# unilight/seq2seq-vc

Measured on AMD Instinct MI355X. Metric: mel-frames/sec (train), higher is better.
Workload: dtype bf16; 1 GPU; VTN egs/arctic/vc1 (vtn.v1.yaml) training step: fwd+Seq2SeqLoss+bwd+clip+Adam+WarmupLR; batch_per_gpu=32, global_batch=32, T_src=256, T_tgt=256, mel_dim=80, parallelism=dp1, split_backward=False, hip_graph=True, backward_stages=1

## Files before the change

### include/s2svc_hip.h

```cpp
#ifndef S2SVC_HIP_H
#define S2SVC_HIP_H
#include <stdint.h>
#ifdef __cplusplus
extern "C" {
#endif

const char* s2svc_last_error(void);
int s2svc_abi_version(void);
int s2svc_launch_floor(int workgroups, int threads, void* sink_1024_words, void* stream);

int s2svc_event_create(void** out );
int s2svc_event_destroy(void* ev);
int s2svc_event_record(void* ev, void* stream);
int s2svc_stream_wait_event(void* stream, void* ev);

enum { S2SVC_LAYOUT_KC = 0,
       S2SVC_LAYOUT_RC = 1 };
enum { S2SVC_OP_DENSE = 0,
       S2SVC_OP_CONV1D = 1,
       S2SVC_OP_CONV2D_S2 = 2,
       S2SVC_OP_TCONV2D_S2 = 3 };

typedef struct {
  const void* ptr;
// ... 116 lines not shown
int s2svc_axpby(int dtype, int64_t n, float a, const void* x, float b, const void* y, void* out, void* stream);
#define S2SVC_SCALAR_TERMS_MAX 8
typedef struct {
  const float* x[S2SVC_SCALAR_TERMS_MAX];
  int32_t n[S2SVC_SCALAR_TERMS_MAX];
  float w[S2SVC_SCALAR_TERMS_MAX];
  int32_t k;
  int32_t reserved_;
} s2svc_scalar_terms;
int s2svc_weighted_sum(const s2svc_scalar_terms* terms , float* out, void* stream);
int s2svc_weighted_sum_bwd(const s2svc_scalar_terms* grads , const float* g, void* stream);
int s2svc_scalars_axpy(const s2svc_scalar_terms* terms , float beta, float* acc, void* stream);
int s2svc_fill_zero(void* p, int64_t nbytes, void* stream);
int s2svc_seed_advance(uint64_t* seed, uint64_t inc, void* stream);
int s2svc_pad_cols(int dtype, int64_t rows, int N, int ldo, const void* in, void* out, void* stream);
int s2svc_decoder_input(int out_dtype, int B, int Tin, int r, int D, int64_t ys_batch_stride, const float* ys, void* out, void* stream);
int s2svc_append_eos(int B, int T, int64_t ldx, const int64_t* xs, const int32_t* lens, int64_t eos, int64_t pad, int64_t* out, void* stream);
int s2svc_copy_rows(int dtype, int64_t rows, int D, int64_t lds, const void* src, void* out, void* stream);
int s2svc_stop_labels(int B, int T, int64_t ld_labels, const float* labels, const int32_t* lens, float* out, void* stream);
int s2svc_add_n(int dtype, int64_t n, int k, const void* x0, const void* x1, const void* x2, const void* x3, void* out, void* stream);
int s2svc_add_head_bias(int dtype, int64_t rows, int D, const void* q, const float* u, const float* v, void* qu, void* qv,
                        void* stream);
int s2svc_add_head_bias_ld(int dtype, int64_t rows, int D, const void* q, int64_t ldq, const float* u, const float* v, void* qu,
                           void* qv, void* stream);
int s2svc_add_rows(int dtype, int64_t rows, int D, const void* a, int64_t lda, const void* b, int64_t ldb, void* out, int64_t ldo,
                   void* stream);
int s2svc_glu_fwd(int dtype, int64_t rows, int C, const void* x, void* y, void* stream);
int s2svc_glu_bwd(int dtype, int64_t rows, int C, const void* x, const void* dy, void* dx, void* stream);
int s2svc_cast(int in_dtype, int out_dtype, int64_t n, const void* x, void* y, void* stream);
int s2svc_gather3(int in_dtype, int out_dtype, int n0, int n1, int n2, int64_t s0, int64_t s1, int64_t s2, int64_t off,
                  const void* in, void* out, void* stream);
typedef struct s2svc_gather3_job {
  const void* in;
  void* out;
  int64_t s0, s1, s2, off;
  int32_t n0, n1, n2;
  int32_t out_dtype;
} s2svc_gather3_job;
int s2svc_gather3_grouped(const s2svc_gather3_job* jobs , int n, void* stream);
enum { S2SVC_DERIVED_GATHER3 = 0, S2SVC_DERIVED_TCONV2D = 1 };
typedef struct s2svc_derived_job {
  const void* in;
  void* out;
  int64_t s0, s1, s2, off;
  int32_t n0, n1, n2;
  int32_t out_dtype;
  int32_t kind;
  int32_t reserved_;
} s2svc_derived_job;
int s2svc_derived_refresh(const s2svc_derived_job* jobs , int n, void* stream);
int s2svc_derived_refresh_plan(const s2svc_derived_job* jobs , int n, int32_t* path , int32_t* units );
int s2svc_permute_inner(int n, int A, int B, const float* src, float* dst, int accumulate, void* stream);
int s2svc_rowscale(int dtype, int64_t rows, int D, const void* x, const float* s, void* out, void* stream);

int s2svc_conv_in1_fwd(int dtype, int B, int Tn, int Fn, int O, const void* x, const float* w, const float* bias, void* y,
                       void* stream);
int s2svc_conv_in1_wgrad(int dtype, int B, int Tn, int Fn, int O, const void* x, const void* dy, const void* y, float* dw,
                         float* db, int accumulate, float* partial, int max_chunks, void* stream);
int s2svc_col2im_s2(int dtype, int B, int T1, int F1, int C, int T2, int F2, const void* dcols, void* dx, void* stream);
int s2svc_interp_nearest(int dtype, int B, int Tin, int Tout, int C, const void* x, void* y, const int32_t* ext_in,
                         const int32_t* ext_out, void* stream);
int s2svc_interp_nearest_bwd(int dtype, int B, int Tin, int Tout, int C, const void* dy, void* dx, const int32_t* ext_in,
                             const int32_t* ext_out, void* stream);
int s2svc_interp_nearest_rows(int dtype, int B, int Tin, int Tout, int C, const void* x, void* y, const int32_t* lens_in,
                              const int32_t* lens_out, void* stream);
int s2svc_dwconv(int dtype, int B, int Tn, int C, int ks, int dil, const void* x, const float* w, const float* bias,
                 void* y, int flip, void* stream);
int s2svc_dwconv_add(int dtype, int B, int Tn, int C, int ks, int dil, const void* x, const float* w, const float* bias,
                     const void* add, void* y, int flip, void* stream);
int s2svc_dwconv_wgrad(int dtype, int B, int Tn, int C, int ks, int dil, const void* x, const void* dy, float* dw,
                       int accumulate, float* ws, int ws_chunks, void* stream);

int s2svc_convmod_supported(int C, int ks);
int s2svc_convmod_fwd(int B, int Tn, int C, int ks, const void* y2, const float* w, const float* bias, void* z, float eps,
                      float momentum, float* mean, float* rstd, float* run_mean, float* run_var, int64_t* num_batches, float* ws,
                      const int32_t* vlens, void* stream);
int s2svc_bn_swish_apply(int64_t rows, int C, const void* z, const float* mean, const float* rstd, const float* gamma,
                         const float* beta, void* out, int Tn, const int32_t* vlens, void* stream);
int s2svc_convmod_bwd(int B, int Tn, int C, int ks, const void* da, const void* z, const void* y2, const float* w, const float* mean,
                      const float* rstd, const float* gamma, const float* beta, void* dy2, float* sdy, float* sdyx,
                      float* dgamma_acc, float* dbeta_acc, float* ws_stats, float* ws_w, const int32_t* vlens, void* stream);
int s2svc_convmod_wgrad_final(int C, int ks, int chunks, const float* ws_w, float* dw, float* db, int accumulate, void* stream);

int s2svc_convmod_infer_supported(int C, int ks);
int s2svc_convmod_infer(int dtype, int B, int Tn, int C, int ks, const void* y2, const float* w, const float* bias, const float* run_mean,
                        const float* run_var, const float* gamma, const float* beta, float eps, void* out, const int32_t* vlens,
                        void* stream);

int s2svc_bn_stats_vec(int rows, int C, const void* x, float eps, float momentum, float* mean, float* rstd, float* run_mean,
                       float* run_var, int64_t* num_batches, float* ws, int Tn, const int32_t* vlens, void* stream);
int s2svc_bn_act_apply_vec(int rows, int C, const void* x, const float* mean, const float* rstd, const float* gamma, const float* beta,
                           int act, float drop_p, const uint64_t* seed_base, uint64_t seed_off, void* y, void* pre_act, int Tn,
                           const int32_t* vlens, void* stream);
int s2svc_bn_act_bwd_vec(int rows, int C, const void* dz, const void* saved, const void* x, const float* mean, const float* rstd,
                         const float* gamma, int act, float drop_p, const uint64_t* seed_base, uint64_t seed_off, void* dx, float* sdy,
                         float* sdyx, float* dgamma_acc, float* dbeta_acc, float* ws, int Tn, const int32_t* vlens, void* stream);

int s2svc_pairwise_l2_logsoftmax(int dtype, int B, int Tf, int Tx, int A, const void* feats, const void* text,
                                 const int32_t* text_lens, float* logp, float* dist, void* stream);
int s2svc_pairwise_l2_bwd_g(int dtype, int B, int Tf, int Tx, const float* logp, const float* dist, const float* dlogp,
                            const int32_t* text_lens, void* G, float* rowsum, void* stream);
int64_t s2svc_mas_ws_bytes(int B, int Tf, int Tx);
int s2svc_mas(int B, int Tf, int Tx, const float* log_p_attn, const int32_t* text_lens, const int32_t* feat_lens,
              int32_t* path, float* ds, float* binmean, void* ws, void* stream);
int s2svc_mas_binloss_bwd(int B, int Tf, int Tx, const int32_t* path, const int32_t* feat_lens, const float* gout,
                          float* dlogp, void* stream);
// ... 189 lines not shown
```

### seq2seq_vc_amd/_lib.py

```python
import ctypes
import os
import subprocess
import sys
from concurrent.futures import ThreadPoolExecutor

_HERE = os.path.dirname(os.path.abspath(__file__))
CSRC = os.path.join(_HERE, "csrc")
LIB_PATH = os.environ.get("S2SVC_LIB") or os.path.join(CSRC, "libs2svc_hip.so")
HIPCC = os.environ.get("HIPCC", "/opt/rocm/bin/hipcc")
ARCH = "gfx950"


def sources():
    return sorted(f for f in os.listdir(CSRC) if f.endswith(".hip"))


DEBUG_EXEC_LIB_PATH = os.path.join(CSRC, "libs2svc_hip_dbgexec.so")


def build_library(force=False, verbose=True, debug_exec=False):
    lib_path = DEBUG_EXEC_LIB_PATH if debug_exec else LIB_PATH
    if not debug_exec and os.environ.get("S2SVC_LIB"):
        lib_path = os.path.join(CSRC, "libs2svc_hip.so")
    srcs = [os.path.join(CSRC, f) for f in sources()]
# ... 40 lines not shown
    deps = [src, os.path.join(_HERE, "..", "include", "s2svc_hip.h")]
    if not force and os.path.exists(TORCH_OPS_LIB_PATH) and os.path.getmtime(TORCH_OPS_LIB_PATH) >= max(os.path.getmtime(p) for p in deps):
        return TORCH_OPS_LIB_PATH
    tlib = E.library_paths()[0]
    cmd = ["g++", "-O2", "-std=c++17", "-fPIC", "-shared", "-D__HIP_PLATFORM_AMD__=1", "-DUSE_ROCM=1",
           f"-D_GLIBCXX_USE_CXX11_ABI={int(torch._C._GLIBCXX_USE_CXX11_ABI)}"]
    cmd += [f"-I{p}" for p in E.include_paths()] + ["-I/opt/rocm/include", src, "-o", TORCH_OPS_LIB_PATH,
                                                    f"-L{tlib}", "-ltorch", "-ltorch_cpu", "-lc10", "-lc10_hip", "-ltorch_hip",
                                                    f"-L{CSRC}", "-ls2svc_hip", "-Wl,-rpath,$ORIGIN", f"-Wl,-rpath,{tlib}"]
    if verbose:
        print("[s2svc build]", " ".join(cmd), file=sys.stderr)
    subprocess.run(cmd, check=True)
    return TORCH_OPS_LIB_PATH


c_i32, c_i64, c_f32, c_u64, c_vp = ctypes.c_int32, ctypes.c_int64, ctypes.c_float, ctypes.c_uint64, ctypes.c_void_p


class Operand(ctypes.Structure):
    _fields_ = [("ptr", c_vp), ("ld", c_i64), ("layout", c_i32), ("mode", c_i32), ("C", c_i32), ("T", c_i32),
                ("pad", c_i32), ("T1", c_i32), ("F1", c_i32), ("T2", c_i32), ("F2", c_i32), ("bs0", c_i64),
                ("bs1", c_i64), ("zero_padded", c_i32), ("reserved_", c_i32)]


class GemmDesc(ctypes.Structure):
    _fields_ = [("A", Operand), ("B", Operand), ("C", c_vp), ("ldc", c_i64), ("cbs0", c_i64), ("cbs1", c_i64),
                ("c_dtype", c_i32), ("bias", c_vp), ("res", c_vp), ("ldr", c_i64), ("rbs0", c_i64), ("rbs1", c_i64),
                ("M", c_i32), ("N", c_i32), ("K", c_i32), ("nb0", c_i32), ("nb1", c_i32), ("act", c_i32),
                ("alpha", c_f32), ("dtype", c_i32), ("accumulate", c_i32), ("splitk", c_i32), ("ws", c_vp),
                ("a_rowsum", c_vp), ("a_rowsum_ws", c_vp), ("a_rowsum_accumulate", c_i32), ("tile_hint", c_i32),
                ("emask", c_vp), ("ldm", c_i64), ("drop_p", c_f32), ("emask_mode", c_i32), ("seed_base", c_vp),
                ("seed_off", c_u64), ("c_map", c_i32), ("cm_T1", c_i32), ("cm_F1", c_i32), ("cm_Tc", c_i32), ("cm_Fc", c_i32),
                ("cm_pt", c_i32), ("cm_pf", c_i32), ("reserved3_", c_i32), ("c_pre", c_vp)]


class ScalarTerms(ctypes.Structure):
    _fields_ = [("x", c_vp * 8), ("n", c_i32 * 8), ("w", c_f32 * 8), ("k", c_i32), ("reserved_", c_i32)]


class Gather3Job(ctypes.Structure):
    _fields_ = [("in_", c_vp), ("out", c_vp), ("s0", c_i64), ("s1", c_i64), ("s2", c_i64), ("off", c_i64), ("n0", c_i32),
                ("n1", c_i32), ("n2", c_i32), ("out_dtype", c_i32)]


class DerivedJob(ctypes.Structure):
    _fields_ = [("in_", c_vp), ("out", c_vp), ("s0", c_i64), ("s1", c_i64), ("s2", c_i64), ("off", c_i64), ("n0", c_i32),
                ("n1", c_i32), ("n2", c_i32), ("out_dtype", c_i32), ("kind", c_i32), ("reserved_", c_i32)]


class ColreduceItem(ctypes.Structure):
    _fields_ = [("dy", c_vp), ("x", c_vp), ("mean", c_vp), ("rstd", c_vp), ("out_sum", c_vp), ("out_dot", c_vp), ("ws", c_vp),
                ("dtype", c_i32), ("rows", c_i32), ("D", c_i32), ("mode", c_i32), ("accumulate", c_i32), ("ws_chunks", c_i32),
                ("scale", c_f32), ("reserved_", c_i32)]


_SIGS = {
    "s2svc_gemm": [ctypes.POINTER(GemmDesc), c_vp],
    "s2svc_gemm_grouped_ok": [c_vp],
    "s2svc_tconv2d_weights": [c_i32, c_i32, c_vp, c_vp, c_vp],
    "s2svc_gemm_grouped": [c_vp, c_i32, c_i32, c_vp],
    "s2svc_gemm_grouped_batched": [c_vp, c_i32, c_vp],
    "s2svc_gemm_wgrad_ok": [c_vp],
    "s2svc_gemm_wgrad_grouped": [c_vp, c_i32, c_vp, c_vp],
    "s2svc_gemm_wgrad_grouped_bg": [c_vp, c_i32, c_vp, c_vp, c_i32],
    "s2svc_gemm_set_w8": [c_i32, c_i32],
    "s2svc_gemm_set_8ph": [c_i32],
    "s2svc_launch_floor": [c_i32, c_i32, c_vp, c_vp],
    "s2svc_event_create": [c_vp],
    "s2svc_event_destroy": [c_vp],
    "s2svc_event_record": [c_vp, c_vp],
    "s2svc_stream_wait_event": [c_vp, c_vp],
    "s2svc_decode_ln_linear_supported": [c_i32, c_i32, c_i32],
    "s2svc_decode_ln_linear": [ctypes.POINTER(GemmDesc), c_vp, c_vp, c_f32, c_vp, c_i64, c_vp],
    "s2svc_length_regulate_index": [c_i32, c_i32, c_i32, c_vp, c_vp, c_vp, c_vp, c_vp],
    "s2svc_length_regulate_fwd": [c_i32, c_i32, c_i32, c_i32, c_i32, c_vp, c_vp, c_f32, c_vp, c_vp],
    "s2svc_length_regulate_bwd": [c_i32, c_i32, c_i32, c_i32, c_i32, c_vp, c_vp, c_vp, c_vp, c_vp],
    "s2svc_attn_durations": [c_i32, c_i32, c_i32, c_vp, c_vp, c_vp, c_vp, c_vp],
    "s2svc_durations_finalize": [c_i32, c_i32, c_i32, c_vp, c_vp, c_f32, c_vp, c_vp, c_vp, c_vp],
    "s2svc_layernorm_fwd": [c_i32, c_i32, c_i32, c_vp, c_vp, c_f32, c_f32, c_vp, c_u64, c_vp, c_vp, c_f32, c_vp, c_vp, c_vp, c_vp, c_vp],
    "s2svc_layernorm_bwd": [c_i32, c_i32, c_i32, c_vp, c_vp, c_vp, c_vp, c_vp, c_vp, c_f32, c_f32, c_vp, c_u64, c_vp, c_vp, c_vp],
    "s2svc_layernorm_bwd_pg_chunks": [c_i32, c_i32, c_i32, c_vp, c_vp, c_vp, c_vp, c_vp, c_vp],
    "s2svc_layernorm_bwd_pg": [c_i32, c_i32, c_i32, c_vp, c_vp, c_vp, c_vp, c_vp, c_vp, c_f32, c_f32, c_vp, c_u64, c_vp, c_vp, c_vp, c_vp],
    "s2svc_colreduce_grouped": [c_vp, c_i32, c_vp],
    "s2svc_colreduce": [c_i32, c_i32, c_i32, c_i32, c_vp, c_vp, c_vp, c_vp, c_f32, c_vp, c_vp, c_i32, c_vp, c_i32, c_i32, c_vp, c_vp],
    "s2svc_bn_finalize": [c_i32, c_i32, c_f32, c_f32, c_vp, c_vp, c_vp, c_vp, c_vp, c_vp, c_i32, c_i32, c_vp, c_vp],
    "s2svc_rstd_from_var": [c_i32, c_f32, c_vp, c_vp, c_vp],
    "s2svc_bn_apply": [c_i32, c_i64, c_i32, c_vp, c_vp, c_vp, c_vp, c_vp, c_i32, c_f32, c_vp, c_u64, c_vp, c_vp, c_i32, c_vp, c_vp],
    "s2svc_bn_bwd": [c_i32, c_i64, c_i32, c_vp, c_vp, c_vp, c_vp, c_vp, c_vp, c_vp, c_i32, c_vp, c_i32, c_vp, c_vp],
    "s2svc_bn_stats": [c_i32, c_i32, c_i32, c_vp, c_f32, c_f32, c_vp, c_vp, c_vp, c_vp, c_vp, c_vp, c_i32, c_i32, c_vp, c_vp],
    "s2svc_attn_softmax_fwd": [c_i32, c_i32, c_i32, c_i32, c_i32, c_i32, c_vp, c_vp, c_i32, c_i32, c_i32, c_f32, c_vp, c_i32, c_f32,
                               c_vp, c_u64, c_vp, c_vp, c_vp],
    "s2svc_attn_softmax_bwd": [c_i32, c_i32, c_i32, c_i32, c_i32, c_i32, c_vp, c_vp, c_vp, c_f32, c_f32, c_vp, c_u64, c_vp, c_vp, c_i32,
                               c_i32, c_i32, c_vp],
    "s2svc_act_dropout_fwd": [c_i32, c_i64, c_vp, c_i32, c_f32, c_vp, c_u64, c_vp, c_vp],
    "s2svc_act_dropout_bwd": [c_i32, c_i64, c_vp, c_vp, c_i32, c_f32, c_vp, c_u64, c_vp, c_vp],
    "s2svc_posenc_fwd": [c_i32, c_i64, c_i32, c_i32, c_vp, c_f32, c_vp, c_vp, c_f32, c_vp, c_u64, c_vp, c_vp],
    "s2svc_posenc_bwd": [c_i32, c_i64, c_i32, c_i32, c_vp, c_f32, c_vp, c_f32, c_vp, c_u64, c_vp, c_vp, c_vp, c_vp],
    "s2svc_axpby": [c_i32, c_i64, c_f32, c_vp, c_f32, c_vp, c_vp, c_vp],
    "s2svc_add_n": [c_i32, c_i64, c_i32, c_vp, c_vp, c_vp, c_vp, c_vp, c_vp],
    "s2svc_weighted_sum": [ctypes.POINTER(ScalarTerms), c_vp, c_vp],
    "s2svc_weighted_sum_bwd": [ctypes.POINTER(ScalarTerms), c_vp, c_vp],
    "s2svc_scalars_axpy": [ctypes.POINTER(ScalarTerms), c_f32, c_vp, c_vp],
    "s2svc_fill_zero": [c_vp, c_i64, c_vp],
    "s2svc_seed_advance": [c_vp, c_u64, c_vp],
    "s2svc_pad_cols": [c_i32, c_i64, c_i32, c_i32, c_vp, c_vp, c_vp],
    "s2svc_decoder_input": [c_i32, c_i32, c_i32, c_i32, c_i32, c_i64, c_vp, c_vp, c_vp],
    "s2svc_stop_labels": [c_i32, c_i32, c_i64, c_vp, c_vp, c_vp, c_vp],
    "s2svc_append_eos": [c_i32, c_i32, c_i64, c_vp, c_vp, c_i64, c_i64, c_vp, c_vp],
    "s2svc_copy_rows": [c_i32, c_i64, c_i32, c_i64, c_vp, c_vp, c_vp],
    "s2svc_add_head_bias": [c_i32, c_i64, c_i32, c_vp, c_vp, c_vp, c_vp, c_vp, c_vp],
    "s2svc_add_head_bias_ld": [c_i32, c_i64, c_i32, c_vp, c_i64, c_vp, c_vp, c_vp, c_vp, c_vp],
    "s2svc_add_rows": [c_i32, c_i64, c_i32, c_vp, c_i64, c_vp, c_i64, c_vp, c_i64, c_vp],
    "s2svc_glu_fwd": [c_i32, c_i64, c_i32, c_vp, c_vp, c_vp],
    "s2svc_glu_bwd": [c_i32, c_i64, c_i32, c_vp, c_vp, c_vp, c_vp],
    "s2svc_cast": [c_i32, c_i32, c_i64, c_vp, c_vp, c_vp],
    "s2svc_gather3_grouped": [c_vp, c_i32, c_vp],
    "s2svc_derived_refresh": [c_vp, c_i32, c_vp],
    "s2svc_derived_refresh_plan": [c_vp, c_i32, c_vp, c_vp],
    "s2svc_permute_inner": [c_i32, c_i32, c_i32, c_vp, c_vp, c_i32, c_vp],
    "s2svc_gather3": [c_i32, c_i32, c_i32, c_i32, c_i32, c_i64, c_i64, c_i64, c_i64, c_vp, c_vp, c_vp],
    "s2svc_mas": [c_i32, c_i32, c_i32, c_vp, c_vp, c_vp, c_vp, c_vp, c_vp, c_vp, c_vp],
    "s2svc_mas_binloss_bwd": [c_i32, c_i32, c_i32, c_vp, c_vp, c_vp, c_vp, c_vp],
    "s2svc_seq_loss_fwd": [c_i32, c_i32, c_i32, c_i32, c_vp, c_vp, c_vp, c_vp, c_vp, c_vp, c_f32, c_vp, c_vp, c_vp],
    "s2svc_seq_loss_bwd": [c_i32, c_i32, c_i32, c_i32, c_vp, c_vp, c_vp, c_vp, c_vp, c_vp, c_f32, c_vp, c_vp, c_vp, c_vp,
                           c_vp, c_vp, c_vp],
    "s2svc_guided_attn_loss_fwd": [c_i32, c_i32, c_i32, c_i32, c_i32, c_vp, c_vp, c_vp, c_f32, c_f32, c_vp, c_vp, c_vp],
    "s2svc_guided_attn_loss_bwd": [c_i32, c_i32, c_i32, c_i32, c_i32, c_vp, c_vp, c_f32, c_f32, c_vp, c_vp, c_vp, c_vp],
    "s2svc_adam_step": [c_i64, c_vp, c_vp, c_vp, c_vp, c_vp, c_f32, c_f32, c_f32, c_f32, c_f32, c_f32, c_vp, c_vp, c_vp],
    "s2svc_transpose_tiles": [c_i64, c_vp, c_vp, c_vp, c_vp],
    "s2svc_col2im_s2": [c_i32, c_i32, c_i32, c_i32, c_i32, c_i32, c_i32, c_vp, c_vp, c_vp],
    "s2svc_interp_nearest": [c_i32, c_i32, c_i32, c_i32, c_i32, c_vp, c_vp, c_vp, c_vp, c_vp],
    "s2svc_interp_nearest_bwd": [c_i32, c_i32, c_i32, c_i32, c_i32, c_vp, c_vp, c_vp, c_vp, c_vp],
    "s2svc_interp_nearest_rows": [c_i32, c_i32, c_i32, c_i32, c_i32, c_vp, c_vp, c_vp, c_vp, c_vp],
    "s2svc_dwconv": [c_i32, c_i32, c_i32, c_i32, c_i32, c_i32, c_vp, c_vp, c_vp, c_vp, c_i32, c_vp],
    "s2svc_dwconv_add": [c_i32, c_i32, c_i32, c_i32, c_i32, c_i32, c_vp, c_vp, c_vp, c_vp, c_vp, c_i32, c_vp],
    "s2svc_dwconv_wgrad": [c_i32, c_i32, c_i32, c_i32, c_i32, c_i32, c_vp, c_vp, c_vp, c_i32, c_vp, c_i32, c_vp],
    "s2svc_convmod_supported": [c_i32, c_i32],
    "s2svc_convmod_fwd": [c_i32, c_i32, c_i32, c_i32, c_vp, c_vp, c_vp, c_vp, c_f32, c_f32, c_vp, c_vp, c_vp, c_vp, c_vp, c_vp, c_vp, c_vp],
    "s2svc_bn_swish_apply": [c_i64, c_i32, c_vp, c_vp, c_vp, c_vp, c_vp, c_vp, c_i32, c_vp, c_vp],
    "s2svc_convmod_bwd": [c_i32, c_i32, c_i32, c_i32, c_vp, c_vp, c_vp, c_vp, c_vp, c_vp, c_vp, c_vp, c_vp, c_vp, c_vp, c_vp, c_vp, c_vp,
                          c_vp, c_vp, c_vp],
    "s2svc_convmod_wgrad_final": [c_i32, c_i32, c_i32, c_vp, c_vp, c_vp, c_i32, c_vp],
    "s2svc_convmod_infer_supported": [c_i32, c_i32],
    "s2svc_convmod_infer": [c_i32, c_i32, c_i32, c_i32, c_i32, c_vp, c_vp, c_vp, c_vp, c_vp, c_vp, c_vp, c_f32, c_vp, c_vp, c_vp],
    "s2svc_bn_stats_vec": [c_i32, c_i32, c_vp, c_f32, c_f32, c_vp, c_vp, c_vp, c_vp, c_vp, c_vp, c_i32, c_vp, c_vp],
    "s2svc_bn_act_apply_vec": [c_i32, c_i32, c_vp, c_vp, c_vp, c_vp, c_vp, c_i32, c_f32, c_vp, c_u64, c_vp, c_vp, c_i32, c_vp, c_vp],
    "s2svc_bn_act_bwd_vec": [c_i32, c_i32, c_vp, c_vp, c_vp, c_vp, c_vp, c_vp, c_i32, c_f32, c_vp, c_u64, c_vp, c_vp, c_vp, c_vp, c_vp, c_vp,
                             c_i32, c_vp, c_vp],
    "s2svc_pairwise_l2_logsoftmax": [c_i32, c_i32, c_i32, c_i32, c_i32, c_vp, c_vp, c_vp, c_vp, c_vp, c_vp],
    "s2svc_pairwise_l2_bwd_g": [c_i32, c_i32, c_i32, c_i32, c_vp, c_vp, c_vp, c_vp, c_vp, c_vp, c_vp],
    "s2svc_rowscale": [c_i32, c_i64, c_i32, c_vp, c_vp, c_vp, c_vp],
    "s2svc_gauss_upsample_probs": [c_i32, c_i32, c_i32, c_i32, c_vp, c_vp, c_vp, c_f32, c_vp, c_vp],
    "s2svc_forward_sum": [c_i32, c_i32, c_i32, c_vp, c_vp, c_vp, c_vp, c_f32, c_vp, c_vp, c_vp, c_vp],
    "s2svc_betabinom_prior": [c_i32, c_i32, c_i32, c_vp, c_vp, c_vp, c_vp],
    "s2svc_conv_in1_fwd": [c_i32, c_i32, c_i32, c_i32, c_i32, c_vp, c_vp, c_vp, c_vp, c_vp],
    "s2svc_conv_in1_wgrad": [c_i32, c_i32, c_i32, c_i32, c_i32, c_vp, c_vp, c_vp, c_vp, c_vp, c_i32, c_vp, c_i32, c_vp],
    "s2svc_attn_fused_supported": [c_i32, c_i32, c_i32, c_i32],
    "s2svc_attn_fused_fwd": [c_i32, c_i32, c_i32, c_i32, c_i32, c_vp, c_i64, c_i64, c_vp, c_i64, c_i64, c_vp, c_i64, c_i64, c_vp, c_i32,
                             c_f32, c_f32, c_vp, c_u64, c_vp, c_i32, c_vp, c_i64, c_i64, c_vp],
    "s2svc_attn_fused_bwd": [c_i32, c_i32, c_i32, c_i32, c_i32, c_vp, c_i64, c_i64, c_vp, c_i64, c_i64, c_vp, c_i64, c_i64, c_vp, c_i64,
                             c_i64, c_vp, c_vp, c_i32, c_f32, c_f32, c_vp, c_u64, c_vp, c_i64, c_i64, c_vp, c_i64, c_i64, c_vp, c_i64,
                             c_i64, c_vp],
    "s2svc_attn_proj_supported": [c_i32, c_i32, c_i32, c_i32, c_i32, c_i32],
    "s2svc_attn_proj_bwd": [c_i32, c_i32, c_i32, c_i32, c_i32, c_vp, c_i64, c_i64, c_vp, c_i64, c_i64, c_vp, c_i64, c_i64, c_vp, c_i64,
                            c_i64, c_vp, c_i64, c_vp, c_vp, c_i32, c_f32, c_f32, c_vp, c_u64, c_vp, c_i64, c_i64, c_vp, c_i64, c_i64,
                            c_vp, c_i64, c_i64, c_vp],
    "s2svc_relattn_supported": [c_i32, c_i32, c_i32, c_i32],
    "s2svc_relattn_fwd": [c_i32, c_i32, c_i32, c_i32, c_vp, c_i64, c_i64, c_vp, c_i64, c_i64, c_vp, c_i64, c_i32, c_vp, c_vp, c_vp, c_f32,
                          c_f32, c_vp, c_u64, c_vp, c_vp, c_i32, c_vp, c_vp, c_vp],
    "s2svc_attn_map_supported": [c_i32, c_i32, c_i32, c_i32],
    "s2svc_attn_map_product_supported": [c_i32],
    "s2svc_attn_map_fwd": [c_i32, c_i32, c_i32, c_i32, c_i32, c_vp, c_i64, c_i64, c_vp, c_i64, c_i64, c_vp, c_i32, c_f32, c_f32, c_vp, c_u64,
# ... 101 lines not shown
```

### seq2seq_vc_amd/ops/functional.py

```python
import math
import os

import torch
from torch.autograd import Function

from . import kernels as K
from . import kernels_attn as KAT

_STATE = {"dtype": torch.float32}


def set_compute_dtype(dtype):
    if dtype not in (torch.float32, torch.bfloat16):
        raise ValueError("compute dtype must be float32 or bfloat16")
    _STATE["dtype"] = dtype


def compute_dtype():
    return _STATE["dtype"]


def to_compute(x):
    return K.cast(x.contiguous(), _STATE["dtype"])

# ... 62 lines not shown
        if name in self.points:
            raise RuntimeError(f"gradient cut '{name}' was reached twice in one forward pass")
        inner = tuple(t.detach().requires_grad_(True) if (t is not None and t.requires_grad) else t for t in xs)
        self.points[name] = (xs, inner)
        return inner if isinstance(x, tuple) else inner[0]

    def resume(self, name):
        outer, inner = self.points.get(name, (None, None))
        if outer is None:
            return
        pairs = [(o, i.grad) for o, i in zip(outer, inner) if o is not None and o.requires_grad and i is not o and i.grad is not None]
        if pairs:
            torch.autograd.backward([o for o, _ in pairs], [g for _, g in pairs], retain_graph=False)

    def clear(self):
        self.points.clear()


_CUTS = {"active": None}


class grad_cuts:
    def __init__(self, cuts):
        self.cuts = cuts

    def __enter__(self):
        self.prev, _CUTS["active"] = _CUTS["active"], self.cuts
        if self.cuts is not None:
            self.cuts.clear()
        return self.cuts

    def __exit__(self, *exc):
        _CUTS["active"] = self.prev
        return False


def cut_point(x, name):
    c = _CUTS["active"]
    return x if c is None else c.cut(x, name)


class _Side:
    enabled = False
    streams = []
    idx = 0
    pending = []
    queue = []
    origins = []
    inline = False
    inline_q = {}
    batch = 16
    grouped = []
    grouped_cr = []
    on_flush = None


def _taken_streams():
    h = {st.cuda_stream for st in _Side.streams}
    if _Branch.stream is not None:
        h.add(_Branch.stream.cuda_stream)
    if torch.cuda.is_available():
        h.add(torch.cuda.current_stream().cuda_stream)
    return h


def distinct_stream(taken=None):
    taken = _taken_streams() if taken is None else set(taken)
    for _ in range(96):
        st = torch.cuda.Stream()
        if st.cuda_stream not in taken:
            return st
    raise RuntimeError("no distinct stream left in torch's stream pool")


def enable_side_streams(n=4, inline_batches=False, batch=None):
    K.set_wgrad_cap(64 if n > 0 else 0)
    _Side.enabled = n > 0
    _Side.inline = (n == 0) and inline_batches
    _Side.batch = int(batch) if batch else (64 if _Side.inline else 16)
    old, others = _Side.streams, _taken_streams() - {st.cuda_stream for st in _Side.streams}
    if n > 0 and len(old) == n and len({st.cuda_stream for st in old}) == n and not ({st.cuda_stream for st in old} & others):
        pass
    else:
        _Side.streams = []
        for _ in range(n):
            _Side.streams.append(distinct_stream())
    _Side.idx = 0


def _side_run(fn, keep=(), solo=False):
    if solo and _Side.enabled and not _Side.inline:
        held, held_o = _Side.queue, _Side.origins
        _Side.queue, _Side.origins = [fn], [torch.cuda.current_stream()]
        _Side.pending.append(keep)
        _side_flush()
        _Side.queue, _Side.origins = held, held_o
        return
    if _Side.inline:
        cur = torch.cuda.current_stream()
        q = _Side.inline_q.setdefault(cur.cuda_stream, (cur, []))[1]
        q.append(fn)
        _Side.pending.append(keep)
        if len(q) >= _Side.batch:
            _inline_flush(cur.cuda_stream)
        return
    if not _Side.enabled:
        fn()
        return
    _Side.queue.append(fn)
    _Side.origins.append(torch.cuda.current_stream())
    _Side.pending.append(keep)
    if len(_Side.queue) >= _Side.batch:
        _side_flush()


def _run_batch(closures):
    with K.record_grouped(_Side.grouped), K.record_colreduce(_Side.grouped_cr):
        for fn in closures:
            fn()
    if _Side.grouped:
        K.flush_grouped(_Side.grouped)
    if _Side.grouped_cr:
        K.flush_colreduce(_Side.grouped_cr)


def _inline_flush(key):
    st, q = _Side.inline_q.pop(key)
    with torch.cuda.stream(st):
        _run_batch(q)
        if _Side.on_flush is not None:
            _Side.on_flush()
    return st


def _side_flush():
    if _Side.inline:
        return
    if not _Side.queue:
        return
    k = _Side.idx % len(_Side.streams)
    st = _Side.streams[k]
    cur = torch.cuda.current_stream().cuda_stream
    if st.cuda_stream == cur or (_Branch.stream is not None and st.cuda_stream == _Branch.stream.cuda_stream):
        st = _Side.streams[k] = distinct_stream()
    _Side.idx += 1
    seen = set()
    for origin in _Side.origins + [torch.cuda.current_stream()]:
        if origin.cuda_stream not in seen:
            seen.add(origin.cuda_stream)
            st.wait_stream(origin)
    _Side.origins = []
    with torch.cuda.stream(st):
        _run_batch(_Side.queue)
        if _Side.on_flush is not None:
            _Side.on_flush()
    _Side.queue = []


_NO_BRANCH = os.environ.get("S2SVC_NO_BRANCH", "0") == "1"


class _Branch:
    stream = None
    active = False
    dirty = False


def branch_run(fn, uses=()):
    if not torch.cuda.is_available() or _NO_BRANCH:
        return fn()
    main = torch.cuda.current_stream()
    if _Branch.stream is None or _Branch.stream.cuda_stream == main.cuda_stream:
        _Branch.stream = distinct_stream()
    _Branch.stream.wait_stream(main)
    for t in uses:
        if isinstance(t, torch.Tensor) and t.is_cuda:
# ... 985 lines not shown

    @staticmethod
    def backward(ctx, dqu, dqv):
        u, v = ctx.params
        dqu, dqv = _c(dqu), _c(dqv)
        dq = K.axpby(1.0, dqu, 1.0, dqv)
        du, dv = _head_bias_grads(u, v, dqu, dqv)
        return dq, du, dv


def add_head_bias(q, u, v):
    return _HeadBias.apply(q, u, v)




class _Conv1d(Function):
    @staticmethod
    def forward(ctx, x, weight, bias, act):
        x = _c(x)
        B, T, Cin = x.shape
        Cout, _, ks = weight.shape
        pad = (ks - 1) // 2
        dtype = x.dtype
        wp = K.gather3_cached(weight, (Cout, ks, Cin), (Cin * ks, 1, ks), 0, dtype)
        y = torch.empty((B, T, Cout), dtype=dtype, device=x.device)
        K.gemm(K.operand(x, Cin, mode=K.CONV1D, C=Cin, T=T, pad=pad), K.operand(wp, ks * Cin), B * T, Cout, ks * Cin, y,
               in_dtype=dtype, bias=bias, act=act)
        ctx.act = act
        ctx.params = (weight, bias)
        ctx.save_for_backward(x, y if act else None)
        return y

    @staticmethod
    def backward(ctx, dy):
        x, y = ctx.saved_tensors
        weight, bias = ctx.params
        B, T, Cin = x.shape
        Cout, _, ks = weight.shape
        pad = (ks - 1) // 2
        dtype = x.dtype
        dy = _c(dy)
        if ctx.act:
            dy = K.act_dropout_bwd(dy, y, act=ctx.act)
        dx = None
        if ctx.needs_input_grad[0]:
            wd = K.gather3_cached(weight, (Cin, ks, Cout), (ks, -1, Cin * ks), ks - 1, dtype)
            dx = torch.empty((B, T, Cin), dtype=dtype, device=x.device)
            K.gemm(K.operand(dy, Cout, mode=K.CONV1D, C=Cout, T=T, pad=pad), K.operand(wd, ks * Cout), B * T, Cin, ks * Cout, dx,
                   in_dtype=dtype)
        dw = db = None
        if weight.requires_grad:
            def work():
                dwp = torch.empty((Cout, ks * Cin), dtype=torch.float32, device=x.device)
                rs, racc, dbv = _bias_sink(bias, Cout)
                tile, sk = K.plan_gemm(Cout, ks * Cin, B * T)
                K.gemm(K.operand(dy, Cout, layout=K.RC), K.operand(x, Cin, layout=K.RC, mode=K.CONV1D, C=Cin, T=T, pad=pad),
                       Cout, ks * Cin, B * T, dwp, in_dtype=dtype, splitk=sk, tile=tile, a_rowsum=rs, a_rowsum_accumulate=racc,
                       wgrad=True)
                return _emit_permuted(weight, dwp, Cout, ks, Cin), dbv
            if _slotted(weight, bias):
                _side_run(work, keep=(dy, x))
            else:
                dw, db = work()
        elif bias is not None and bias.requires_grad:
            db, _ = _reduce_to(bias, None, 0, dy.view(B * T, Cout))
        return dx, dw, db, None


class _CropRows(Function):

    @staticmethod
    def forward(ctx, x, vlens):
        from . import kernels_sdp as KS
        ctx.vlens = vlens
        return KS.mask_rows(_c(x), vlens)

    @staticmethod
    def backward(ctx, dy):
        from . import kernels_sdp as KS
        return KS.mask_rows(_c(dy), ctx.vlens), None


def crop_rows(x, vlens):
    return x if vlens is None else _CropRows.apply(x, vlens)


def conv1d(x, weight, bias=None, act=None, vlens=None):
    if vlens is not None and weight.shape[-1] > 1:
        x = crop_rows(x, vlens)
    return _Conv1d.apply(x, weight, bias, act)






class _Conv2dS2(Function):
    @staticmethod
    def forward(ctx, x, weight, bias, grad_premasked=False, input_is_relu=False):
        x = _c(x)
        ctx.grad_premasked = grad_premasked
        ctx.input_is_relu = input_is_relu
        B, T1, F1, C = x.shape
        O = weight.shape[0]
        T2, F2 = (T1 - 3) // 2 + 1, (F1 - 3) // 2 + 1
# ... 349 lines not shown
```

### seq2seq_vc_amd/ops/kernels.py

```python
import ctypes
import math
import os

import torch

from .. import _lib

KC, RC = 0, 1
DENSE, CONV1D, CONV2D_S2, TCONV2D_S2 = 0, 1, 2, 3
ACT = {None: 0, "none": 0, "relu": 1, "tanh": 2, "swish": 3, "sigmoid": 4, "gelu": 5}

_DT = {torch.float32: 0, torch.bfloat16: 1}


def dt(t):
    try:
        return _DT[t.dtype if isinstance(t, torch.Tensor) else t]
    except KeyError:
        raise TypeError(f"unsupported dtype {t.dtype if isinstance(t, torch.Tensor) else t}")


def ptr(t):
    return None if t is None else t.data_ptr()

# ... 444 lines not shown
    nws = L.s2svc_gemm_wgrad_ws_floats(ctypes.addressof(arr), len(descs))
    ws = torch.empty(nws, dtype=torch.float32, device=torch.cuda.current_device()) if nws else None
    if capped and _W8_CAP[0] > 0:
        _lib.check(L.s2svc_gemm_wgrad_grouped_bg(ctypes.addressof(arr), len(descs), ptr(ws), stream(), _W8_CAP[0]),
                   "s2svc_gemm_wgrad_grouped_bg")
        return
    _lib.check(L.s2svc_gemm_wgrad_grouped(ctypes.addressof(arr), len(descs), ptr(ws), stream()), "s2svc_gemm_wgrad_grouped")


def launch_group_batched(descs):
    if not descs:
        return
    if len(descs) > 1:
        arr = (_lib.GemmDesc * len(descs))(*descs)
        rc = _lib.lib().s2svc_gemm_grouped_batched(ctypes.addressof(arr), len(descs), stream())
        if rc == 0:
            return
        if rc != 1:
            _lib.check(rc, "s2svc_gemm_grouped_batched")
    for d in descs:
        _lib.check(_lib.lib().s2svc_gemm(ctypes.byref(d), stream()), "s2svc_gemm")


def flush_grouped(queue):
    pending = list(queue)
    del queue[:]
    while pending:
        seen, group, rest = set(), [], []
        for d in pending:
            keys = {d.C} | ({d.a_rowsum} if d.a_rowsum else set())
            if keys & seen:
                rest.append(d)
            else:
                seen |= keys
                group.append(d)
        pending = rest
        L = _lib.lib()
        w8 = [d for d in group if L.s2svc_gemm_wgrad_ok(ctypes.addressof(d))]
        if w8:
            group = [d for d in group if not any(d is w for w in w8)]
            if _Audit.on:
                _audit_write("grouped weight gradient (W8)", *[d.C for d in w8], *[d.a_rowsum for d in w8])
            launch_wgrad_group(w8)
        big = [d for d in group if _GROUP_TILE == 64 and ((d.M + 127) // 128) * ((d.N + 127) // 128) >= _GROUP_BIG_TILES]
        small = [d for d in group if not any(d is b for b in big)]
        for part, tile in ((big, 128), (small, _GROUP_TILE)):
            if part:
                arr = (_lib.GemmDesc * len(part))(*part)
                if _Audit.on:
                    _audit_write("grouped weight gradient", *[d.C for d in part], *[d.a_rowsum for d in part])
                _lib.check(_lib.lib().s2svc_gemm_grouped(ctypes.addressof(arr), len(part), tile, stream()), "s2svc_gemm_grouped")


def layernorm_fwd(x, gamma, beta, eps, res=None, p=0.0, seed=(None, 0), need_stats=True, hscale=1.0):
    _need_cuda(x)
    D = x.shape[-1]
    rows = x.numel() // D
    y = torch.empty_like(x)
    s = torch.empty_like(x) if res is not None else None
    mean = torch.empty(rows, dtype=torch.float32, device=x.device) if need_stats else None
    rstd = torch.empty(rows, dtype=torch.float32, device=x.device) if need_stats else None
    _lib.check(_lib.lib().s2svc_layernorm_fwd(dt(x), rows, D, ptr(x), ptr(res), p, hscale, seed[0], seed[1], ptr(gamma), ptr(beta),
                                              eps, ptr(y), ptr(s), ptr(mean), ptr(rstd), stream()), "layernorm_fwd")
    return y, s, mean, rstd


def layernorm_bwd(dy, s, mean, rstd, gamma, ds_extra=None, p=0.0, seed=(None, 0), want_dh=False, hscale=1.0, want_partials=False,
                  partials_ok=True):
    D = s.shape[-1]
    rows = s.numel() // D
    ds = torch.empty_like(s)
    dh = torch.empty_like(s) if want_dh else None
    L = _lib.lib()
    if want_partials and partials_ok:
        chunks = L.s2svc_layernorm_bwd_pg_chunks(dt(s), rows, D, ptr(dy), ptr(s), ptr(gamma), ptr(ds_extra), ptr(ds), ptr(dh))
        if chunks > 0:
            ws = torch.empty(chunks * 2 * D, dtype=torch.float32, device=s.device)
            _lib.check(L.s2svc_layernorm_bwd_pg(dt(s), rows, D, ptr(dy), ptr(s), ptr(mean), ptr(rstd), ptr(gamma), ptr(ds_extra), p,
                                                hscale, seed[0], seed[1], ptr(ds), ptr(dh), ptr(ws), stream()), "layernorm_bwd_pg")
            return ds, dh, (ws, chunks)
    _lib.check(L.s2svc_layernorm_bwd(dt(s), rows, D, ptr(dy), ptr(s), ptr(mean), ptr(rstd), ptr(gamma),
                                     ptr(ds_extra), p, hscale, seed[0], seed[1], ptr(ds), ptr(dh), stream()),
               "layernorm_bwd")
    return (ds, dh, None) if want_partials else (ds, dh)


def colreduce_partials(ws, chunks, D, out_sum, out_dot):
    it = _lib.ColreduceItem()
    it.dy, it.x, it.mean, it.rstd = None, None, None, None
    it.out_sum, it.out_dot, it.ws = ptr(out_sum), ptr(out_dot), ptr(ws)
    it.dtype, it.rows, it.D, it.mode, it.accumulate, it.ws_chunks, it.scale = _DT[torch.float32], chunks, D, 7, 1, chunks, 1.0
    if _CR_RECORDER is not None:
        _CR_RECORDER.append((it, (out_sum, out_dot, ws)))
        return
    if _Audit.on:
        _audit_write("column reduction", ptr(out_sum), ptr(out_dot))
    arr = (_lib.ColreduceItem * 1)(it)
    _lib.check(_lib.lib().s2svc_colreduce_grouped(ctypes.addressof(arr), 1, stream()), "colreduce_grouped")


_WS_CHUNKS = 64


def colreduce(mode, dy, x=None, mean=None, rstd=None, scale=1.0, want_dot=False, rows=None, D=None, out_sum=None,
              out_dot=None, accumulate=False, vlens=None, Tn=0):
    t = dy if dy is not None else x
# ... 486 lines not shown
```

Measured before the change: 1.732 million mel-frames/sec.

## Add grouped direct conv1d weight-gradient MFMA kernel accumulating into grad slots

Adds a dedicated HIP kernel that computes ks=5 bf16 conv1d weight gradients directly from dy and x tiles in LDS, using transposed LDS reads and MFMA, and accumulates into the fp32 grad slot in the final layout. Conv1d weight-gradient closures on side batches are queued and flushed as one grouped launch, replacing the generic im2col-style GEMM plus permute and temp buffer. This removes the extra workspace, the permute pass and per-layer launches. In exchange the dw update is a plain non-atomic read-add-write, and the path applies only to bias-free, slotted, 16-aligned shapes.

```diff
diff --git a/include/s2svc_hip.h b/include/s2svc_hip.h
--- a/include/s2svc_hip.h
+++ b/include/s2svc_hip.h
@@ -192,6 +192,17 @@
 int s2svc_derived_refresh_plan(const s2svc_derived_job* jobs , int n, int32_t* path , int32_t* units );
 int s2svc_permute_inner(int n, int A, int B, const float* src, float* dst, int accumulate, void* stream);
 int s2svc_rowscale(int dtype, int64_t rows, int D, const void* x, const float* s, void* out, void* stream);
+typedef struct s2svc_conv1d_wgrad_item {
+  const void* dy;
+  const void* x;
+  float* dw;
+  int32_t B, T, Cin, Cout, ks;
+  int32_t dtype;
+  int32_t chunk_steps;
+  int32_t reserved_;
+} s2svc_conv1d_wgrad_item;
+int s2svc_conv1d_wgrad_supported(int Cout, int Cin, int ks, int dtype);
+int s2svc_conv1d_wgrad_grouped(const s2svc_conv1d_wgrad_item* items , int n, int max_workgroups, void* stream);
 
 int s2svc_conv_in1_fwd(int dtype, int B, int Tn, int Fn, int O, const void* x, const float* w, const float* bias, void* y,
                        void* stream);
diff --git a/seq2seq_vc_amd/_lib.py b/seq2seq_vc_amd/_lib.py
--- a/seq2seq_vc_amd/_lib.py
+++ b/seq2seq_vc_amd/_lib.py
@@ -116,6 +116,11 @@
     _fields_ = [("dy", c_vp), ("x", c_vp), ("mean", c_vp), ("rstd", c_vp), ("out_sum", c_vp), ("out_dot", c_vp), ("ws", c_vp),
                 ("dtype", c_i32), ("rows", c_i32), ("D", c_i32), ("mode", c_i32), ("accumulate", c_i32), ("ws_chunks", c_i32),
                 ("scale", c_f32), ("reserved_", c_i32)]
+
+
+class Conv1dWgradItem(ctypes.Structure):
+    _fields_ = [("dy", c_vp), ("x", c_vp), ("dw", c_vp), ("B", c_i32), ("T", c_i32), ("Cin", c_i32), ("Cout", c_i32), ("ks", c_i32),
+                ("dtype", c_i32), ("chunk_steps", c_i32), ("reserved_", c_i32)]
 
 
 _SIGS = {
@@ -182,6 +187,8 @@
     "s2svc_derived_refresh": [c_vp, c_i32, c_vp],
     "s2svc_derived_refresh_plan": [c_vp, c_i32, c_vp, c_vp],
     "s2svc_permute_inner": [c_i32, c_i32, c_i32, c_vp, c_vp, c_i32, c_vp],
+    "s2svc_conv1d_wgrad_supported": [c_i32, c_i32, c_i32, c_i32],
+    "s2svc_conv1d_wgrad_grouped": [c_vp, c_i32, c_i32, c_vp],
     "s2svc_gather3": [c_i32, c_i32, c_i32, c_i32, c_i32, c_i64, c_i64, c_i64, c_i64, c_vp, c_vp, c_vp],
     "s2svc_mas": [c_i32, c_i32, c_i32, c_vp, c_vp, c_vp, c_vp, c_vp, c_vp, c_vp, c_vp],
     "s2svc_mas_binloss_bwd": [c_i32, c_i32, c_i32, c_vp, c_vp, c_vp, c_vp, c_vp],
diff --git a/seq2seq_vc_amd/csrc/conv1d_wgrad.hip b/seq2seq_vc_amd/csrc/conv1d_wgrad.hip
--- /dev/null
+++ b/seq2seq_vc_amd/csrc/conv1d_wgrad.hip
@@ -0,0 +1,216 @@
+#include "common.h"
+
+#include "../../include/s2svc_hip.h"
+
+namespace {
+
+typedef __attribute__((ext_vector_type(4))) float f32x4_t;
+typedef __attribute__((ext_vector_type(8))) __bf16 bf16x8_t;
+typedef __attribute__((ext_vector_type(4))) short s16x4_t;
+typedef __attribute__((ext_vector_type(8))) short s16x8_t;
+typedef __attribute__((address_space(3))) s16x4_t lds_s16x4_t;
+
+constexpr int CW_MAX_ITEMS = 16;
+constexpr int CW_ROWS = 64;
+constexpr int CW_BLK = 64;
+
+struct cw_item {
+  const bf16_t* dy;
+  const bf16_t* x;
+  float* dw;
+  int B, T, Cin, Cout;
+  int unit0, nci;
+  int chunk;
+};
+struct cw_args {
+  cw_item it[CW_MAX_ITEMS];
+  int n, units;
+};
+
+template <int KS>
+struct cw_geom {
+  static constexpr int PAD = (KS - 1) / 2;
+  static constexpr int XROWS = CW_ROWS + KS - 1;
+  static constexpr int DY_SUB = CW_ROWS * 32 + 64;
+  static constexpr int X_SUB = XROWS * 32 + 64;
+  static constexpr int X_OFF = 4 * DY_SUB;
+  static constexpr int BYTES = 4 * DY_SUB + 4 * X_SUB;
+  static constexpr int XEXTRA = (XROWS - 64) * 8;
+};
+
+__device__ __forceinline__ bf16x8_t cw_fragment(const char* img, int row0, int lane) {
+  const char* p = img + (row0 + (lane >> 4) * 4 + ((lane & 15) >> 2)) * 32 + (lane & 3) * 8;
+  const s16x4_t lo = __builtin_amdgcn_ds_read_tr16_b64_v4i16((lds_s16x4_t*)p);
+  const s16x4_t hi = __builtin_amdgcn_ds_read_tr16_b64_v4i16((lds_s16x4_t*)(p + 512));
+  const s16x8_t v = {lo[0], lo[1], lo[2], lo[3], hi[0], hi[1], hi[2], hi[3]};
+  return __builtin_bit_cast(bf16x8_t, v);
+}
+
+template <int KS>
+__global__ __launch_bounds__(256) void conv1d_wgrad_kernel(const cw_args a) {
+  typedef cw_geom<KS> G;
+  __shared__ __attribute__((aligned(256))) char smem[G::BYTES];
+  const int tid = threadIdx.x, lane = tid & 63, wave = tid >> 6;
+  const int wm = (wave >> 1) * 32, wn = (wave & 1) * 32;
+  const int pc = tid & 7, pr = tid >> 3;
+  const int st_off = pr * 32 + (pc & 1) * 16;
+
+  for (int u = blockIdx.x; u < a.units; u += gridDim.x) {
+    int ii = 0;
+#pragma unroll 1
+    for (int q = 1; q < a.n; ++q)
+      if (u >= a.it[q].unit0) ii = q;
+    const cw_item& it = a.it[ii];
+    const int lu = u - it.unit0;
+    const int o0 = (lu / it.nci) * CW_BLK, c0 = (lu % it.nci) * CW_BLK;
+    const int T = it.T, Cin = it.Cin, Cout = it.Cout;
+    const int tsteps = (T + CW_ROWS - 1) / CW_ROWS, nsteps = it.B * tsteps;
+    const bool dy_col = o0 + pc * 8 < Cout, x_col = c0 + pc * 8 < Cin;
+    const bf16_t* dyp = it.dy + o0 + pc * 8;
+    const bf16_t* xp = it.x + c0 + pc * 8;
+
+    f32x4_t acc[KS][2][2], tot[KS][2][2];
+#pragma unroll
+    for (int j = 0; j < KS; ++j)
+#pragma unroll
+      for (int fm = 0; fm < 2; ++fm)
+#pragma unroll
+        for (int fn = 0; fn < 2; ++fn) acc[j][fm][fn] = tot[j][fm][fn] = (f32x4_t){0.f, 0.f, 0.f, 0.f};
+    int run_end = it.chunk > 0 && it.chunk < nsteps ? it.chunk : nsteps;
+
+    uint4 rdy[2], rx[3];
+    auto fetch = [&](int s) {
+      const int b = s / tsteps, t0 = (s - b * tsteps) * CW_ROWS;
+      const int64_t row0 = (int64_t)b * T;
+#pragma unroll
+      for (int h = 0; h < 2; ++h) {
+        const int t = t0 + pr + h * 32;
+        rdy[h] = (dy_col && t < T) ? *reinterpret_cast<const uint4*>(dyp + (row0 + t) * Cout) : make_uint4(0u, 0u, 0u, 0u);
+      }
+#pragma unroll
+      for (int h = 0; h < 3; ++h) {
+        const int t = t0 - G::PAD + pr + h * 32;
+        const bool mine = h < 2 || tid < G::XEXTRA;
+        rx[h] = (mine && x_col && t >= 0 && t < T) ? *reinterpret_cast<const uint4*>(xp + (row0 + t) * Cin) : make_uint4(0u, 0u, 0u, 0u);
+      }
+    };
+
+    fetch(0);
+    for (int s = 0; s < nsteps; ++s) {
+      __syncthreads();
+      {
+        char* dimg = smem + (pc >> 1) * G::DY_SUB + st_off;
+        char* ximg = smem + G::X_OFF + (pc >> 1) * G::X_SUB + st_off;
+        *reinterpret_cast<uint4*>(dimg) = rdy[0];
+        *reinterpret_cast<uint4*>(dimg + 32 * 32) = rdy[1];
+        *reinterpret_cast<uint4*>(ximg) = rx[0];
+        *reinterpret_cast<uint4*>(ximg + 32 * 32) = rx[1];
+        if (tid < G::XEXTRA) *reinterpret_cast<uint4*>(ximg + 64 * 32) = rx[2];
+      }
+      __syncthreads();
+      const int tleft = T - (s % tsteps) * CW_ROWS;
+      if (s + 1 < nsteps) fetch(s + 1);
+      const int halves = tleft > 32 ? 2 : 1;
+      for (int kh = 0; kh < halves; ++kh) {
+        bf16x8_t fa[2];
+#pragma unroll
+        for (int fm = 0; fm < 2; ++fm) fa[fm] = cw_fragment(smem + ((wm >> 4) + fm) * G::DY_SUB, kh * 32, lane);
+#pragma unroll
+        for (int j = 0; j < KS; ++j) {
+          bf16x8_t fb[2];
+#pragma unroll
+          for (int fn = 0; fn < 2; ++fn) fb[fn] = cw_fragment(smem + G::X_OFF + ((wn >> 4) + fn) * G::X_SUB, kh * 32 + j, lane);
+#pragma unroll
+          for (int fm = 0; fm < 2; ++fm)
+#pragma unroll
+            for (int fn = 0; fn < 2; ++fn)
+              acc[j][fm][fn] = __builtin_amdgcn_mfma_f32_16x16x32_bf16(fa[fm], fb[fn], acc[j][fm][fn], 0, 0, 0);
+        }
+      }
+      if (s + 1 == run_end) {
+#pragma unroll
+        for (int j = 0; j < KS; ++j)
+#pragma unroll
+          for (int fm = 0; fm < 2; ++fm)
+#pragma unroll
+            for (int fn = 0; fn < 2; ++fn) {
+#pragma unroll
+              for (int e = 0; e < 4; ++e) tot[j][fm][fn][e] += acc[j][fm][fn][e];
+              acc[j][fm][fn] = (f32x4_t){0.f, 0.f, 0.f, 0.f};
+            }
+        run_end = run_end + it.chunk < nsteps ? run_end + it.chunk : nsteps;
+      }
+    }
+
+#pragma unroll
+    for (int fm = 0; fm < 2; ++fm)
+#pragma unroll
+      for (int fn = 0; fn < 2; ++fn) {
+        const int ci = c0 + wn + fn * 16 + (lane & 15);
+#pragma unroll
+        for (int e = 0; e < 4; ++e) {
+          const int o = o0 + wm + fm * 16 + (lane >> 4) * 4 + e;
+          if (o < Cout && ci < Cin) {
+            float* p = it.dw + ((int64_t)o * Cin + ci) * KS;
+#pragma unroll
+            for (int j = 0; j < KS; ++j) p[j] += tot[j][fm][fn][e];
+          }
+        }
+      }
+  }
+}
+
+bool cw_supported(int Cout, int Cin, int ks, int dtype) {
+  return dtype == S2S_BF16 && ks == 5 && Cout >= 16 && Cin >= 16 && (Cout % 16) == 0 && (Cin % 16) == 0;
+}
+
+}
+
+extern "C" int s2svc_conv1d_wgrad_supported(int Cout, int Cin, int ks, int dtype) { return cw_supported(Cout, Cin, ks, dtype) ? 1 : 0; }
+
+extern "C" int s2svc_conv1d_wgrad_grouped(const s2svc_conv1d_wgrad_item* items, int n, int max_workgroups, void* stream) {
+  S2S_REQUIRE(items != nullptr && n >= 1, "conv1d_wgrad_grouped: no items");
+  S2S_REQUIRE(max_workgroups >= 0, "conv1d_wgrad_grouped: max_workgroups must be >= 0");
+  for (int i = 0; i < n; ++i) {
+    const s2svc_conv1d_wgrad_item& p = items[i];
+    S2S_REQUIRE(cw_supported(p.Cout, p.Cin, p.ks, p.dtype), "conv1d_wgrad_grouped: unsupported item (bf16, ks 5, Cin and Cout multiples of 16)");
+    S2S_REQUIRE(p.chunk_steps >= 0, "conv1d_wgrad_grouped: chunk_steps must be >= 0");
+    S2S_REQUIRE(p.B >= 1 && p.T >= 1 && (int64_t)p.B * p.T < (1ll << 31), "conv1d_wgrad_grouped: bad B / T");
+    S2S_REQUIRE(p.dy != nullptr && p.x != nullptr && p.dw != nullptr, "conv1d_wgrad_grouped: null operand");
+    S2S_REQUIRE((reinterpret_cast<uintptr_t>(p.dy) & 15) == 0 && (reinterpret_cast<uintptr_t>(p.x) & 15) == 0,
+                "conv1d_wgrad_grouped: dy and x must be 16-byte aligned");
+    S2S_REQUIRE((reinterpret_cast<uintptr_t>(p.dw) & 3) == 0, "conv1d_wgrad_grouped: dw must be 4-byte aligned");
+  }
+  int i = 0;
+  while (i < n) {
+    cw_args a;
+    uintptr_t dw_bytes[CW_MAX_ITEMS];
+    a.n = 0;
+    a.units = 0;
+    for (; i < n && a.n < CW_MAX_ITEMS; ++i) {
+      const s2svc_conv1d_wgrad_item& p = items[i];
+      const uintptr_t lo = reinterpret_cast<uintptr_t>(p.dw), hi = lo + (uintptr_t)p.Cout * p.Cin * p.ks * 4;
+      bool clash = false;
+      for (int q = 0; q < a.n; ++q) {
+        const uintptr_t qlo = reinterpret_cast<uintptr_t>(a.it[q].dw);
+        const uintptr_t qhi = qlo + dw_bytes[q];
+        clash = clash || (lo < qhi && qlo < hi);
+      }
+      if (clash) break;
+      dw_bytes[a.n] = hi - lo;
+      cw_item& c = a.it[a.n++];
+      c.dy = static_cast<const bf16_t*>(p.dy);
+      c.x = static_cast<const bf16_t*>(p.x);
+      c.dw = p.dw;
+      c.B = p.B; c.T = p.T; c.Cin = p.Cin; c.Cout = p.Cout;
+      c.unit0 = a.units;
+      c.nci = (p.Cin + CW_BLK - 1) / CW_BLK;
+      c.chunk = p.chunk_steps;
+      a.units += c.nci * ((p.Cout + CW_BLK - 1) / CW_BLK);
+    }
+    const int grid = (max_workgroups > 0 && max_workgroups < a.units) ? max_workgroups : a.units;
+    hipLaunchKernelGGL(conv1d_wgrad_kernel<5>, dim3(grid), dim3(256), 0, static_cast<hipStream_t>(stream), a);
+    S2S_CHECK_LAUNCH("conv1d_wgrad_kernel");
+  }
+  return 0;
+}
diff --git a/seq2seq_vc_amd/ops/functional.py b/seq2seq_vc_amd/ops/functional.py
--- a/seq2seq_vc_amd/ops/functional.py
+++ b/seq2seq_vc_amd/ops/functional.py
@@ -138,6 +138,7 @@
     batch = 16
     grouped = []
     grouped_cr = []
+    grouped_c1w = []
     on_flush = None
 
 
@@ -201,13 +202,15 @@
 
 
 def _run_batch(closures):
-    with K.record_grouped(_Side.grouped), K.record_colreduce(_Side.grouped_cr):
+    with K.record_grouped(_Side.grouped), K.record_colreduce(_Side.grouped_cr), K.record_conv1d_wgrad(_Side.grouped_c1w):
         for fn in closures:
             fn()
     if _Side.grouped:
         K.flush_grouped(_Side.grouped)
     if _Side.grouped_cr:
         K.flush_colreduce(_Side.grouped_cr)
+    if _Side.grouped_c1w:
+        K.flush_conv1d_wgrad(_Side.grouped_c1w, K.get_wgrad_cap())
 
 
 def _inline_flush(key):
@@ -1299,6 +1302,9 @@
         dw = db = None
         if weight.requires_grad:
             def work():
+                if (K.get_wgrad_cap() > 0 and _slotted(weight) and K.conv1d_wgrad_enabled()
+                        and K.conv1d_wgrad_supported(Cout, Cin, ks, dtype, bias) and K.conv1d_wgrad_queue(dy, x, weight._s2s_grad)):
+                    return None, None
                 dwp = torch.empty((Cout, ks * Cin), dtype=torch.float32, device=x.device)
                 rs, racc, dbv = _bias_sink(bias, Cout)
                 tile, sk = K.plan_gemm(Cout, ks * Cin, B * T)
diff --git a/seq2seq_vc_amd/ops/kernels.py b/seq2seq_vc_amd/ops/kernels.py
--- a/seq2seq_vc_amd/ops/kernels.py
+++ b/seq2seq_vc_amd/ops/kernels.py
@@ -520,6 +520,87 @@
                 _lib.check(_lib.lib().s2svc_gemm_grouped(ctypes.addressof(arr), len(part), tile, stream()), "s2svc_gemm_grouped")
 
 
+_C1W_RECORDER = None
+
+
+class record_conv1d_wgrad:
+
+    def __init__(self, queue):
+        self.queue = queue
+
+    def __enter__(self):
+        global _C1W_RECORDER
+        self.prev, _C1W_RECORDER = _C1W_RECORDER, self.queue
+        return self.queue
+
+    def __exit__(self, *exc):
+        global _C1W_RECORDER
+        _C1W_RECORDER = self.prev
+        return False
+
+
+def conv1d_wgrad_enabled():
+    return os.environ.get("S2SVC_NO_CONV1D_WGRAD", "0") != "1"
+
+
+def conv1d_wgrad_supported(Cout, Cin, ks, dtype, bias=None):
+    if bias is not None or dtype not in _DT:
+        return False
+    return bool(_lib.lib().s2svc_conv1d_wgrad_supported(int(Cout), int(Cin), int(ks), _DT[dtype]))
+
+
+def conv1d_wgrad_queue(dy, x, dw):
+    if _C1W_RECORDER is None:
+        return False
+    _C1W_RECORDER.append((dy, x, dw))
+    return True
+
+
+def _c1w_item(dy, x, dw):
+    _need_cuda(dy)
+    if dy.dim() != 3 or x.dim() != 3 or dy.shape[:2] != x.shape[:2] or not dy.is_contiguous() or not x.is_contiguous() or dy.dtype != x.dtype:
+        raise TypeError("conv1d_wgrad: dy (B, T, Cout) and x (B, T, Cin) must be contiguous tensors of one dtype and one (B, T)")
+    (B, T, Cout), Cin = dy.shape, x.shape[2]
+    if dw.dtype != torch.float32 or not dw.is_contiguous() or dw.numel() % (Cout * Cin) or dw.device != dy.device:
+        raise TypeError("conv1d_wgrad: dw must be a contiguous fp32 tensor of Cout * Cin * ks elements on the operands' device")
+    it = _lib.Conv1dWgradItem()
+    it.dy, it.x, it.dw = ptr(dy), ptr(x), ptr(dw)
+    it.B, it.T, it.Cin, it.Cout, it.ks, it.dtype = B, T, Cin, Cout, dw.numel() // (Cout * Cin), dt(dy)
+    it.chunk_steps = conv1d_wgrad_chunk(B, T, Cin, Cout, it.ks)
+    return it
+
+
+def conv1d_wgrad_chunk(B, T, Cin, Cout, ks):
+    if T % 64:
+        return 0
+    ktiles = B * T // 64
+    sk = max(1, plan_gemm(Cout, ks * Cin, B * T)[1])
+    return (ktiles + sk - 1) // sk if sk > 1 else 0
+
+
+def conv1d_wgrad_grouped(items, cap=0):
+    pending = [(_c1w_item(*t), t) for t in items]
+    while pending:
+        seen, group, rest = set(), [], []
+        for it, keep in pending:
+            if it.dw in seen:
+                rest.append((it, keep))
+            else:
+                seen.add(it.dw)
+                group.append((it, keep))
+        pending = rest
+        arr = (_lib.Conv1dWgradItem * len(group))(*[g[0] for g in group])
+        if _Audit.on:
+            _audit_write("grouped conv1d weight gradient", *[g[0].dw for g in group])
+        _lib.check(_lib.lib().s2svc_conv1d_wgrad_grouped(ctypes.addressof(arr), len(group), int(cap), stream()), "s2svc_conv1d_wgrad_grouped")
+
+
+def flush_conv1d_wgrad(queue, cap=0):
+    items = list(queue)
+    del queue[:]
+    conv1d_wgrad_grouped(items, cap)
+
+
 def layernorm_fwd(x, gamma, beta, eps, res=None, p=0.0, seed=(None, 0), need_stats=True, hscale=1.0):
     _need_cuda(x)
     D = x.shape[-1]
```

After: 1.752 million mel-frames/sec (median of 6 runs). 1.2% higher.
